# JingyunLiang/HCFlow

Hardware: AMD Instinct MI355X
Metric: HR images/sec (inverse sample) DIV2K x4 160px LR (higher is better)
Workload: dtype f32 via f16x3 split (hi/lo f16 products, f32 accumulate); 1 GPU; SR_DF2K_4X inverse sampling (netG reverse=True), batch 16/GPU, LR 160x160 -> HR 640x640, tau=0.8, eps on device, output all-gather over RCCL for N>1; global_batch=16, lr_size=160, parallelism=dp1, streams_per_gpu=2

## Files before the change

hcflow_amd/csrc/hcf_conv_wino.h:

```cpp
#pragma once
#include <hip/hip_runtime.h>
#include <stdint.h>
#include <string.h>
#include <math.h>
#include <type_traits>
#include <vector>

namespace hcf {
namespace wino {

constexpr int TW = 32, TH = 8, HWP = TW + 2, HHP = TH + 2;
constexpr int A_REAL_PIECES = HHP * HWP * 4;
constexpr int A_BYTES = 22 * 1024;
constexpr int W_BYTES = 16 * 2 * 2 * 32 * 16;
constexpr int STAGE = A_BYTES + W_BYTES;
constexpr int X_BYTES = 10240;
constexpr int S0_OFF = 0, X_OFF = STAGE, S1_OFF = STAGE + X_BYTES, TAB_OFF = S1_OFF + STAGE;
constexpr int LDS_BYTES = TAB_OFF + 512;
constexpr float UNSPLIT = 1.f / 2048.f;

struct Src { const float* p; int cs, c0, n; };
struct Args {
  Src src[3];
  int nsrc;
// ... 48 lines not shown
          memcpy(&pk[o], &p0, 2);
          memcpy(&pk[o + 512], &p1, 2);
        }
    }
  return true;
}

constexpr int W4_BYTES = 65536;
static inline bool pack_weights_wino64(const float* w, int cin, int cout, std::vector<uint16_t>& pk) {
#pragma clang fp contract(off)
  static const double G[4][3] = {{1, 0, 0}, {.5, .5, .5}, {.5, -.5, .5}, {0, 0, 1}};
  if (cout != 64 || (cin & 15)) return false;
  const int nchunk = cin / 16;
  pk.assign(((size_t)nchunk + 1) * (W4_BYTES / 2), 0);
  for (int oc = 0; oc < cout; ++oc)
    for (int ic = 0; ic < cin; ++ic) {
      const float* g = w + ((size_t)oc * cin + ic) * 9;
      double t[4][3], U[4][4];
      for (int i = 0; i < 4; ++i)
        for (int j = 0; j < 3; ++j) t[i][j] = G[i][0] * g[0 * 3 + j] + G[i][1] * g[1 * 3 + j] + G[i][2] * g[2 * 3 + j];
      for (int i = 0; i < 4; ++i)
        for (int j = 0; j < 4; ++j) U[i][j] = t[i][0] * G[j][0] + t[i][1] * G[j][1] + t[i][2] * G[j][2];
      const int nt = oc >> 5, n = oc & 31, c = ic >> 4, h = (ic >> 3) & 1, e = ic & 7;
      for (int xi = 0; xi < 4; ++xi)
        for (int nu = 0; nu < 4; ++nu) {
          const double u = U[xi][nu] * ((xi == 2) ? -1.0 : 1.0) * ((nu == 2) ? -1.0 : 1.0);
          const float x = (float)u;
          if (!(fabsf(x) * 2048.f < 60000.f)) return false;
          const _Float16 hi = (_Float16)x;
          const _Float16 p0 = (_Float16)((float)hi * 2048.f), p1 = (_Float16)((float)((u - (double)(float)hi) * 2048.0));
          const size_t o = (size_t)c * (W4_BYTES / 2) + (size_t)(((xi * 4 + nu) * 2 + nt) * 2) * 512 + (size_t)h * 256 + (size_t)n * 8 + e;
          memcpy(&pk[o], &p0, 2);
          memcpy(&pk[o + 512], &p1, 2);
        }
    }
  return true;
}

constexpr int F1_BYTES = 16384;
static inline bool pack_weights_1x1_frag(const float* w, std::vector<uint16_t>& pk) {
  pk.assign(F1_BYTES / 2, 0);
  for (int mt = 0; mt < 2; ++mt)
    for (int ks = 0; ks < 4; ++ks)
      for (int ln = 0; ln < 64; ++ln)
        for (int e = 0; e < 8; ++e) {
          const int oc = mt * 32 + (ln & 31), ic = 16 * ks + 8 * (ln >> 5) + e;
          const float x = w[oc * 64 + ic];
          if (!(fabsf(x) * 2048.f < 60000.f)) return false;
          const _Float16 hi = (_Float16)x;
          const _Float16 p0 = (_Float16)((float)hi * 2048.f), p1 = (_Float16)((x - (float)hi) * 2048.f);
          const size_t o = ((size_t)((mt * 4 + ks) * 2 + 0) * 64 + ln) * 8 + e;
          memcpy(&pk[o], &p0, 2);
          memcpy(&pk[o + 512], &p1, 2);
        }
  return true;
}

#if defined(__HIPCC__)
typedef float f32x16 __attribute__((ext_vector_type(16)));
typedef float f32x4 __attribute__((ext_vector_type(4)));
typedef _Float16 f16x8 __attribute__((ext_vector_type(8)));
typedef const char __attribute__((address_space(1)))* gcptr;
typedef __attribute__((address_space(3))) void* lptr;

__device__ __forceinline__ int xcd_remap(int orig, int n) {
  const int xcd = orig & 7, q = n >> 3, r = n & 7;
  const int base = (xcd < r) ? xcd * (q + 1) : r * (q + 1) + (xcd - r) * q;
  return base + (orig >> 3);
}
__device__ __forceinline__ gcptr uniform_ptr(const void* p) {
  const uint64_t v = reinterpret_cast<uint64_t>(p);
  const uint32_t lo = __builtin_amdgcn_readfirstlane((uint32_t)v);
  const uint32_t hi = __builtin_amdgcn_readfirstlane((uint32_t)(v >> 32));
  return (gcptr)(((uint64_t)hi << 32) | lo);
}
__device__ __forceinline__ void glds16(gcptr g, char* lds_wave_base) {
  __builtin_amdgcn_global_load_lds((const __attribute__((address_space(1))) void*)g, (lptr)lds_wave_base, 16, 0, 0);
}
__device__ __forceinline__ float act1(float v, float slope, float lo) { return !(v <= 0.f) ? v : slope * fmaxf(v, lo); }
__device__ __forceinline__ int a_off(int px, int part) {
  const int R = px >> 2, sl = (px & 3) * 4 + part;
  return R * 256 + ((sl ^ ((R & 7) << 1)) << 4);
}


namespace v2 {
constexpr int TH2 = 16, HH2 = TH2 + 2;
constexpr int A2_REAL = HH2 * HWP * 4;
constexpr int A2_BYTES = 39 * 1024;
constexpr int STAGE2 = A2_BYTES + W_BYTES;
constexpr int TAB2_OFF = 2 * STAGE2;
constexpr int LDS2_BYTES = TAB2_OFF + 512;
constexpr int FB2_OFF = LDS2_BYTES;
constexpr int LDS2S_BYTES = FB2_OFF + 512 * 16 + 64;
constexpr int ROWB = HWP * 64;
__host__ __device__ constexpr int a2_off(int row, int x, int part) {
  return row * ROWB + (x >> 2) * 256 + (((((x & 3) * 4 + part)) ^ ((x >> 2) & 7)) << 4);
}
}

typedef _Float16 f16x2 __attribute__((ext_vector_type(2)));
typedef uint32_t u32x4 __attribute__((ext_vector_type(4)));
__device__ __forceinline__ void split8(const float (&v)[8], u32x4& h, u32x4& l) {
#pragma unroll
  for (int i = 0; i < 4; ++i) {
    const f16x2 hh = {(_Float16)v[2 * i], (_Float16)v[2 * i + 1]};
    h[i] = __builtin_bit_cast(uint32_t, hh);
    uint32_t lo;
    asm("v_fma_mixlo_f16 %0, %1, -1.0, %2 op_sel_hi:[1,0,0]" : "=v"(lo) : "v"(h[i]), "v"(v[2 * i]));
    asm("v_fma_mixhi_f16 %0, %1, -1.0, %2 op_sel:[1,0,0] op_sel_hi:[1,0,0]" : "+v"(lo) : "v"(h[i]), "v"(v[2 * i + 1]));
    l[i] = lo;
  }
}

__device__ __forceinline__ void split8s(const float (&v)[8], const float s, u32x4& h, u32x4& l) {
#pragma unroll
  for (int i = 0; i < 4; ++i) {
    uint32_t hi, lo;
    asm("v_fma_mixlo_f16 %0, %1, %2, 0 op_sel_hi:[0,0,0]" : "=v"(hi) : "v"(v[2 * i]), "v"(s));
    asm("v_fma_mixhi_f16 %0, %1, %2, 0 op_sel_hi:[0,0,0]" : "+v"(hi) : "v"(v[2 * i + 1]), "v"(s));
    asm("v_fma_mixlo_f16 %0, %1, %2, -%3 op_sel_hi:[0,0,1]" : "=v"(lo) : "v"(v[2 * i]), "v"(s), "v"(hi));
    asm("v_fma_mixhi_f16 %0, %1, %2, -%3 op_sel:[0,0,1] op_sel_hi:[0,0,1]" : "+v"(lo) : "v"(v[2 * i + 1]), "v"(s), "v"(hi));
    h[i] = hi;
    l[i] = lo;
  }
}
__device__ __forceinline__ void input_scales(const float* in_max, float& in_s, float& out_s, int& in_max_bits) {
  in_s = 1.f; out_s = 1.f;
  in_max_bits = __builtin_amdgcn_readfirstlane(__builtin_bit_cast(int, *in_max));
  const float mx = __builtin_bit_cast(float, in_max_bits);
  if (mx > 0.f && mx < 3.0e38f) {
    int ex = 0;
    (void)frexpf(mx, &ex);
    in_s = ldexpf(1.f, 10 - ex);
    out_s = ldexpf(1.f, ex - 10);
  }
  in_s = __builtin_bit_cast(float, __builtin_amdgcn_readfirstlane(__builtin_bit_cast(int, in_s)));
  out_s = __builtin_bit_cast(float, __builtin_amdgcn_readfirstlane(__builtin_bit_cast(int, out_s)));
}

typedef uint32_t u32x2 __attribute__((ext_vector_type(2)));
__device__ __forceinline__ void split4(const f32x4& v, u32x2& h, u32x2& l) {
#pragma unroll
  for (int i = 0; i < 2; ++i) {
    const f16x2 hh = {(_Float16)v[2 * i], (_Float16)v[2 * i + 1]};
    h[i] = __builtin_bit_cast(uint32_t, hh);
    uint32_t lo;
    asm("v_fma_mixlo_f16 %0, %1, -1.0, %2 op_sel_hi:[1,0,0]" : "=v"(lo) : "v"(h[i]), "v"(v[2 * i]));
    asm("v_fma_mixhi_f16 %0, %1, -1.0, %2 op_sel:[1,0,0] op_sel_hi:[1,0,0]" : "+v"(lo) : "v"(h[i]), "v"(v[2 * i + 1]));
    l[i] = lo;
  }
}

template <int RES, bool SC = false>
__global__ __launch_bounds__(512, 1) void conv_wino2_kernel(const Args a, const int nunits) {
  using namespace v2;
  extern __shared__ __attribute__((aligned(16))) char lds[];
  const int tid = threadIdx.x, lane = tid & 63, half = lane >> 5, li = lane & 31;
  const int wave = __builtin_amdgcn_readfirstlane(tid >> 6);
  const int xp = wave & 1, tg = wave >> 1;
  const int H = a.H, W = a.W, ntn = a.ntile_n, nchunk = a.nchunk;
  const int tiles_x = (W + TW - 1) / TW, tiles_y = (H + TH2 - 1) / TH2;

  const bool w7 = (wave == 7);
  const int padpix = a.B * H * W;
  int upix[5];
#pragma unroll
  for (int j = 0; j < 5; ++j) upix[j] = padpix;
  uint32_t partpk = 0;
#pragma unroll
  for (int j = 0; j < 5; ++j) {
    const int pa_ = (8 * j + wave) * 64 + lane, hy_ = (pa_ * 241) >> 15, q_ = pa_ - hy_ * 136, m_ = q_ >> 4;
    partpk |= (uint32_t)(((q_ & 15) ^ (m_ & 7)) & 3) << (4 + 2 * j);
  }
  const int k0 = __builtin_amdgcn_readfirstlane(a.src[0].n >> 4);
  const int k1 = k0 + __builtin_amdgcn_readfirstlane(a.nsrc > 1 ? (a.src[1].n >> 4) : 0);
  const long long npx = (long long)a.B * H * W;
  const __amdgpu_buffer_rsrc_t rs0 = __builtin_amdgcn_make_buffer_rsrc((void*)a.src[0].p, 0, (int)(npx * a.src[0].cs * 4), 0x00020000);
  const __amdgpu_buffer_rsrc_t rs1 = __builtin_amdgcn_make_buffer_rsrc((void*)a.src[a.nsrc > 1 ? 1 : 0].p, 0, (int)(npx * a.src[a.nsrc > 1 ? 1 : 0].cs * 4), 0x00020000);
  const __amdgpu_buffer_rsrc_t rs2 = __builtin_amdgcn_make_buffer_rsrc((void*)a.src[a.nsrc > 2 ? 2 : 0].p, 0, (int)(npx * a.src[a.nsrc > 2 ? 2 : 0].cs * 4), 0x00020000);
  const __amdgpu_buffer_rsrc_t rsw = __builtin_amdgcn_make_buffer_rsrc((void*)a.wpack, 0, (ntn * nchunk + 1) * W_BYTES, 0x00020000);
  const int csb0 = __builtin_amdgcn_readfirstlane(a.src[0].cs) * 4, csb1 = __builtin_amdgcn_readfirstlane(a.src[1].cs) * 4,
            csb2 = __builtin_amdgcn_readfirstlane(a.src[2].cs) * 4;
  const int cb0 = __builtin_amdgcn_readfirstlane(a.src[0].c0) * 4, cb1 = __builtin_amdgcn_readfirstlane(a.src[1].c0) * 4,
            cb2 = __builtin_amdgcn_readfirstlane(a.src[2].c0) * 4;
  const int wvo = lane * 16;

  int ub = 0, uy0 = 0, ux0 = 0, unt = 0, uc = 0;
#define W2_SETUP_UNIT(U)                                                                           \
  {                                                                                                \
    const int v_ = a.rev ? nunits - 1 - xcd_remap((U), nunits) : xcd_remap((U), nunits);           \
    unt = __builtin_amdgcn_readfirstlane(v_ % ntn);                                                \
    const int t_ = v_ / ntn;                                                                       \
    ux0 = __builtin_amdgcn_readfirstlane((t_ % tiles_x) * TW);                                     \
    uy0 = __builtin_amdgcn_readfirstlane(((t_ / tiles_x) % tiles_y) * TH2);                        \
    ub = __builtin_amdgcn_readfirstlane(t_ / (tiles_x * tiles_y));                                 \
    uc = 0;                                                                                        \
    int ln_ = lane;                                                                                \
    asm volatile("" : "+v"(ln_));                                                                  \
    _Pragma("unroll") for (int j = 0; j < 5; ++j) {                                                \
      const int pa_ = (8 * j + wave) * 64 + ln_;            \
      const int hy_ = (pa_ * 241) >> 15;                                \
      const int q_ = pa_ - hy_ * 136, m_ = q_ >> 4;                                                \
      const int hx_ = m_ * 4 + (((q_ & 15) ^ (m_ & 7)) >> 2);                                      \
      const int y = uy0 + hy_ - 1, x = ux0 + hx_ - 1;                                              \
      upix[j] = (hy_ < HH2 && y >= 0 && y < H && x >= 0 && x < W) ? (ub * H + y) * W + x : padpix; \
    }                                                                                              \
  }
#define W2_DMA(RS, VOFF, SOFF, DST) __builtin_amdgcn_raw_ptr_buffer_load_lds((RS), (lptr)(DST), 16, (VOFF), (SOFF), 0, 0)
  int csb_ = 0, so_ = 0, ws_ = 0;
  uint32_t pp_ = partpk;
  __amdgpu_buffer_rsrc_t rsa_ = rs0;
#define W2_CHUNK_SCALARS()                                                                         \
  {                                                                                                \
    const int sidx_ = (uc < k0) ? 0 : (uc < k1) ? 1 : 2;                                           \
    csb_ = sidx_ == 0 ? csb0 : sidx_ == 1 ? csb1 : csb2;                                           \
    rsa_ = sidx_ == 0 ? rs0 : sidx_ == 1 ? rs1 : rs2;                                              \
    so_ = (sidx_ == 0 ? cb0 + uc * 64 : sidx_ == 1 ? cb1 + (uc - k0) * 64 : cb2 + (uc - k1) * 64); \
    ws_ = (unt * nchunk + uc) * W_BYTES;                                                           \
    pp_ = partpk;                                                                                  \
    asm volatile("" : "+v"(pp_));            \
  }
#define W2_A_SLOT(J, DST)                                                                          \
  {                                                                                                \
    const int p16_ = (int)((pp_ >> (2 * (J))) & 0x30u);                                            \
    const int vo_ = (int)__umul24((unsigned)upix[J], (unsigned)csb_) + p16_;                       \
    W2_DMA(rsa_, vo_, so_, DST);                                                                   \
  }
#define W2_ISSUE(J0, J1, STG)                                                                      \
  {                                                                                                \
    char* const sb_ = lds + (STG) * STAGE2 + wave * 1024;                                          \
    _Pragma("unroll") for (int j_ = (J0); j_ < (J1); ++j_) {                                       \
      if (j_ < 4) W2_A_SLOT(j_ < 5 ? j_ : 0, sb_ + j_ * 8192)                                      \
      else if (j_ == 4) { if (!w7) W2_A_SLOT(4, sb_ + 4 * 8192) else W2_DMA(rsw, wvo, ws_, sb_ + 4 * 8192); } \
      else if (j_ < 8) W2_DMA(rsw, wvo, ws_ + (8 * j_ + wave - 39) * 1024, sb_ + j_ * 8192);       \
      else if (!w7) W2_DMA(rsw, wvo, ws_ + (8 * 8 + wave - 39) * 1024, sb_ + 8 * 8192);            \
    }                                                                                              \
  }

  const int trow = li >> 4, tcol = li & 15;
  int poff[4];
#pragma unroll
  for (int j = 0; j < 4; ++j) poff[j] = a2_off(4 * tg + 2 * trow, 2 * tcol + j, 2 * half);
  const int rowP = xp ? ROWB : 0, rowS = xp ? 3 * ROWB : 2 * ROWB;
  const float sg = __builtin_bit_cast(float, __builtin_amdgcn_readfirstlane(__builtin_bit_cast(int, xp ? -1.f : 1.f)));
  const int fw = A2_BYTES + half * 512 + li * 16 + xp * (8 * 4 * 512);

  float in_s = 1.f, out_s = 1.f;
  int in_max_bits = 0;
  if (SC) input_scales(a.in_max, in_s, out_s, in_max_bits);
  constexpr bool FBK = SC && RES == 0;
  const bool fb = FBK && a.fb_y != nullptr;
  if (tid < 64) {
    const float sc_ = (tid < 32 * ntn) ? a.scale[tid] : 1.f, bi_ = (tid < 32 * ntn) ? a.bias[tid] : 0.f;
    reinterpret_cast<float*>(lds + TAB2_OFF)[tid] = bi_ * sc_;
    reinterpret_cast<float*>(lds + TAB2_OFF)[64 + tid] = sc_ * UNSPLIT * out_s;
  }
  if (FBK) {
    if (fb) {
      *reinterpret_cast<f32x4*>(lds + FB2_OFF + tid * 16) = f32x4{0.f, 0.f, 0.f, 0.f};
      if (tid == 0) *reinterpret_cast<int*>(lds + FB2_OFF + 512 * 16) = 0;
    }
  }
  int u = blockIdx.x;
  if (u >= nunits) return;
#if defined(WINO_PROF)
  unsigned long long pw[8] = {0, 0, 0, 0, 0, 0, 0, 0};
  const unsigned long long pw_t0 = __builtin_readcyclecounter();
#endif
  W2_SETUP_UNIT(u)
  W2_CHUNK_SCALARS()
  W2_ISSUE(0, 9, 0)
  ++uc;
  int g = 0;
  const float slope = a.act == 1 ? 0.f : a.act == 2 ? 0.2f : 1.f;

  while (true) {
    f32x16 acc[8];
#pragma unroll
    for (int p = 0; p < 8; ++p)
#pragma unroll
      for (int r = 0; r < 16; ++r) acc[p][r] = 0.f;
    const int eb = ub, ey0 = uy0, ex0 = ux0, ent = unt;
    const int un = u + gridDim.x;

    for (int c = 0; c < nchunk; ++c, ++g) {
      const int stg = g & 1;
#if defined(WINO_PROF)
      const unsigned long long q0 = __builtin_readcyclecounter();
#endif
      asm volatile("s_waitcnt vmcnt(0)" ::: "memory");
#if defined(WINO_PROF)
      const unsigned long long q1 = __builtin_readcyclecounter();
#endif
      __builtin_amdgcn_s_barrier();
#if defined(WINO_PROF)
      const unsigned long long q2 = __builtin_readcyclecounter();
      pw[0] += q1 - q0; pw[1] += q2 - q1;
#endif
      if (c + 1 == nchunk) {
        if (un < nunits) W2_SETUP_UNIT(un)
        else {
          uc = 0; unt = 0;
#pragma unroll
          for (int j = 0; j < 5; ++j) upix[j] = padpix;
        }
      }
      W2_CHUNK_SCALARS()
      const char* const sb = lds + stg * STAGE2;
      const int so = stg ^ 1;
#define W2_LOAD_ROW(D, OFF)                                                                        \
  _Pragma("unroll") for (int j = 0; j < 4; ++j) {                                                  \
    const f32x4 x0_ = *reinterpret_cast<const f32x4*>(sb + poff[j] + (OFF));                       \
    const f32x4 x1_ = *reinterpret_cast<const f32x4*>(sb + (poff[j] ^ 16) + (OFF));                \
    _Pragma("unroll") for (int k = 0; k < 4; ++k) { D[j][k] = x0_[k]; D[j][4 + k] = x1_[k]; }      \
  }
#define W2_V(NU, T, K) (((NU) == 0) ? T[0][K] - T[2][K] : ((NU) == 1) ? T[1][K] + T[2][K] : ((NU) == 2) ? T[1][K] - T[2][K] : T[1][K] - T[3][K])
#define W2_MFMA(P, WW, VX) acc[P] = __builtin_amdgcn_mfma_f32_32x32x16_f16(WW, __builtin_bit_cast(f16x8, VX), acc[P], 0, 0, 0);
#define W2_XI(I, T)                                                                                \
  _Pragma("unroll") for (int nu = 0; nu < 4; ++nu) {                                               \
    float v_[8];                                                                                   \
    _Pragma("unroll") for (int k = 0; k < 8; ++k) v_[k] = W2_V(nu, T, k);                          \
    u32x4 vh_, vl_;                                                                                \
    if (SC) split8s(v_, in_s, vh_, vl_); else split8(v_, vh_, vl_);                                \
    const f16x8 w1_ = *reinterpret_cast<const f16x8*>(sb + fw + (((I) * 4 + nu) * 4) * 512);       \
    const f16x8 w2_ = *reinterpret_cast<const f16x8*>(sb + fw + (((I) * 4 + nu) * 4 + 2) * 512);   \
    W2_MFMA((I) * 4 + nu, w1_, vh_)                                                                \
    W2_MFMA((I) * 4 + nu, w2_, vh_)                                                                \
    W2_MFMA((I) * 4 + nu, w1_, vl_)                                                                \
  }
      float t_[4][8];
      {
        float ra[4][8], rc[4][8];
        W2_LOAD_ROW(ra, rowP)
        W2_LOAD_ROW(rc, 2 * ROWB)
        W2_ISSUE(0, 3, so)
#pragma unroll
        for (int j = 0; j < 4; ++j)
#pragma unroll
          for (int k = 0; k < 8; ++k) t_[j][k] = ra[j][k] - rc[j][k];
      }
      W2_XI(0, t_)
      W2_ISSUE(3, 6, so)
      {
        float ra[4][8], rc[4][8];
        W2_LOAD_ROW(ra, ROWB)
        W2_LOAD_ROW(rc, rowS)
#pragma unroll
        for (int j = 0; j < 4; ++j)
#pragma unroll
          for (int k = 0; k < 8; ++k) t_[j][k] = fmaf(sg, rc[j][k], ra[j][k]);
      }
      W2_ISSUE(6, 9, so)
      ++uc;
      W2_XI(1, t_)
#if defined(WINO_PROF)
      pw[6] += __builtin_readcyclecounter() - q2;
#endif
#undef W2_XI
#undef W2_MFMA
#undef W2_V
#undef W2_LOAD_ROW
    }

#if defined(WINO_PROF)
    const unsigned long long qe0 = __builtin_readcyclecounter();
#endif
    float chk = 0.f;
    f32x4 fbs = {0.f, 0.f, 0.f, 0.f};
    float fbm = 0.f;
    const float fb_neg = a.fb_act == 1 ? 0.f : a.fb_act == 2 ? 0.2f : 1.f;
    {
      char* const xbuf = lds + ((g - 1) & 1) * STAGE2 + tg * 16384;
      const int p8 = lane >> 3, qd = (lane >> 1) & 3, hd = lane & 1;
      const int wpos = (half * 32 + ((li + 4 * half) & 31)) * 16;
      const int wpos1 = (half * 32 + ((li + 4 * half + 8) & 31)) * 16;
      const int cb = ent * 32 + 8 * qd + 4 * hd;
      const f32x4 bs = *reinterpret_cast<const f32x4*>(lds + TAB2_OFF + cb * 4);
      const f32x4 ms = *reinterpret_cast<const f32x4*>(lds + TAB2_OFF + 256 + cb * 4);
      const bool second = (RES == 0) && a.out2 != nullptr && cb >= a.out2_split;
      const float slope_l = second ? (a.act2 == 1 ? 0.f : a.act2 == 2 ? 0.2f : 1.f) : slope;
      __builtin_amdgcn_s_barrier();
#pragma unroll
      for (int oa = 0; oa < 2; ++oa) {
        f32x4 rv1[2][2], rv2[2][2];
        size_t pixs[2][2];
        bool oks[2][2];
        int rpos[2];
#pragma unroll
        for (int sgrp = 0; sgrp < 2; ++sgrp) {
          const int patch = 16 * xp + 8 * sgrp + p8, prow = patch >> 4, pcol = patch & 15;
          rpos[sgrp] = (hd * 32 + ((patch + 4 * hd + 8 * (qd & 1)) & 31)) * 16 + qd * 1024;
#pragma unroll
          for (int ob = 0; ob < 2; ++ob) {
            const int yy = ey0 + 4 * tg + 2 * prow + oa, xx = ex0 + 2 * pcol + ob;
            oks[sgrp][ob] = yy < H && xx < W;
            pixs[sgrp][ob] = (size_t)((size_t)eb * H + (yy < H ? yy : H - 1)) * W + (xx < W ? xx : W - 1);
            if (RES == 1 || RES == 2) rv1[sgrp][ob] = *reinterpret_cast<const f32x4*>(a.res1 + pixs[sgrp][ob] * a.res1_cs + a.res1_c0 + cb);
            if (RES == 2) rv2[sgrp][ob] = *reinterpret_cast<const f32x4*>(a.res2 + pixs[sgrp][ob] * a.res2_cs + a.res2_c0 + cb);
            if (RES == 3) rv1[sgrp][ob] = *reinterpret_cast<const f32x4*>(a.pre + pixs[sgrp][ob] * a.pre_cs + a.pre_c0 + cb);
            if (FBK) { if (fb) rv1[sgrp][ob] = *reinterpret_cast<const f32x4*>(a.fb_y + pixs[sgrp][ob] * a.fb_y_cs + a.fb_y_c0 + cb); }
          }
        }
        if (oa == 1) __builtin_amdgcn_s_barrier();
#pragma unroll
        for (int q = 0; q < 4; ++q) {
          f32x4 P[2];
#pragma unroll
          for (int e = 0; e < 4; ++e) {
            const int r = 4 * q + e;
            float R[2][2];
#pragma unroll
            for (int i = 0; i < 2; ++i) {
              R[i][0] = acc[i * 4 + 0][r] + acc[i * 4 + 1][r] + acc[i * 4 + 2][r];
              R[i][1] = acc[i * 4 + 1][r] - acc[i * 4 + 2][r] - acc[i * 4 + 3][r];
            }
#pragma unroll
            for (int bb = 0; bb < 2; ++bb)
              P[bb][e] = (oa == 0) ? (xp ? R[0][bb] : R[0][bb] + R[1][bb]) : (xp ? -R[0][bb] - R[1][bb] : R[1][bb]);
          }
          char* const wbq = xbuf + ((xp * 2) * 4 + q) * 1024 + ((q & 1) ? wpos1 : wpos);
          *reinterpret_cast<f32x4*>(wbq) = P[0];
          *reinterpret_cast<f32x4*>(wbq + 4096) = P[1];
        }
        __builtin_amdgcn_s_barrier();
#pragma unroll
        for (int sgrp = 0; sgrp < 2; ++sgrp)
#pragma unroll
          for (int ob = 0; ob < 2; ++ob) {
            const f32x4 y0 = *reinterpret_cast<const f32x4*>(xbuf + ((0 * 2 + ob) * 4) * 1024 + rpos[sgrp]);
            const f32x4 y1 = *reinterpret_cast<const f32x4*>(xbuf + ((1 * 2 + ob) * 4) * 1024 + rpos[sgrp]);
            f32x4 v;
#pragma unroll
            for (int e = 0; e < 4; ++e) {
              const float yv = y0[e] + y1[e];
              chk = fmaf(yv, 0.f, chk);
              float z = fmaf(yv, ms[e], bs[e]);
              if (RES == 3) z = fmaf(rv1[sgrp][ob][e], ms[e] * 2048.f, z);
              v[e] = fmaxf(z, slope_l * z);
              if (RES == 1 || RES == 2) v[e] = fmaf(v[e], a.rs1, rv1[sgrp][ob][e]);
              if (RES == 2) v[e] = fmaf(v[e], a.rs2, rv2[sgrp][ob][e]);
            }
            if (FBK) {
              if (fb && oks[sgrp][ob] && cb < a.cout) {
#pragma unroll
                for (int e = 0; e < 4; ++e) {
                  const float yv = rv1[sgrp][ob][e];
                  const bool pos = a.fb_act == 1 ? (yv > 0.f) : (yv >= 0.f);
                  const float dz = (a.fb_act == 0 || pos) ? v[e] : v[e] * fb_neg;
                  v[e] = dz;
                  fbs[e] += dz;
                  fbm = fmaxf(fbm, fabsf(dz));
                }
              }
            }
            if (oks[sgrp][ob] && cb < a.cout) {
              if (second) *reinterpret_cast<f32x4*>(a.out2 + pixs[sgrp][ob] * a.out2_cs + a.out2_c0 + (cb - a.out2_split)) = v;
              else *reinterpret_cast<f32x4*>(a.out + pixs[sgrp][ob] * a.out_cs + a.out_c0 + cb) = v;
            }
          }
      }
    }
    if (__any(chk != chk)) {
      if (lane == 0) atomicOr(a.ovf, 1 | (2 << (eb % 30)));
    }
    if (FBK) {
      if (fb) {
        f32x4* const slot = reinterpret_cast<f32x4*>(lds + FB2_OFF + tid * 16);
        *slot = *slot + fbs;
        if (fbm > 0.f) atomicMax(reinterpret_cast<int*>(lds + FB2_OFF + 512 * 16), __builtin_bit_cast(int, fbm));
      }
    }
#if defined(WINO_PROF)
    pw[3] += __builtin_readcyclecounter() - qe0;
#endif
    u = un;
    if (u >= nunits) break;
  }
  if (FBK) {
    if (fb) {
      asm volatile("s_waitcnt lgkmcnt(0)\n\ts_barrier" ::: "memory");
      if (tid < 32) {
        const int q4 = tid >> 2, e = tid & 3;
        float t0 = 0.f;
        for (int j = 0; j < 64; ++j) t0 += reinterpret_cast<const float*>(lds + FB2_OFF)[(j * 8 + q4) * 4 + e];
        if (tid < a.cout) {
          a.fb_part[((size_t)blockIdx.x * 2 + 0) * a.cout + tid] = t0;
          a.fb_part[((size_t)blockIdx.x * 2 + 1) * a.cout + tid] = 0.f;
        }
      }
      if (tid == 0) {
        const int m = *reinterpret_cast<const int*>(lds + FB2_OFF + 512 * 16), m2 = max(m, in_max_bits);
        if (a.fb_max && m) atomicMax(reinterpret_cast<int*>(a.fb_max), m);
        if (a.fb_max2 && m2) atomicMax(reinterpret_cast<int*>(a.fb_max2), m2);
      }
    }
  }
#if defined(WINO_PROF)
  if (a.dbg && lane == 0 && (blockIdx.x & 31) == 17) {
    atomicAdd(a.dbg + 0, pw[0]); atomicAdd(a.dbg + 1, pw[1]); atomicAdd(a.dbg + 2, __builtin_readcyclecounter() - pw_t0);
    atomicAdd(a.dbg + 3, pw[3]); atomicAdd(a.dbg + 4, 1ull); atomicAdd(a.dbg + 5, pw[5]); atomicAdd(a.dbg + 6, pw[6]);
  }
#endif
#undef W2_SETUP_UNIT
#undef W2_DMA
#undef W2_A_SLOT
#undef W2_ISSUE
#undef W2_CHUNK_SCALARS
}

namespace v4 {
constexpr int TH4 = 8, HH4 = TH4 + 2;
constexpr int A4_BYTES = 22 * 1024;
constexpr int W4L_BYTES = 48 * 1024;
constexpr int W4_OFF0 = 2 * A4_BYTES;
constexpr int X4_SPARE = 19 * 1024;
constexpr int W4_OFF1 = W4_OFF0 + W4L_BYTES + X4_SPARE;
constexpr int TAB4_OFF = W4_OFF1 + W4L_BYTES;
constexpr int LDS4_BYTES = TAB4_OFF + 1024;
constexpr int NPIECE4 = 22 + 48;
}

template <int RES>
__device__ __forceinline__ void wino64_epilogue(const Args& a, char* const lds, const int tab_off, char* const xbase, f32x16 (&acc)[4][2],
                                                const int eb, const int ey0, const int ex0, const int H, const int W, const float slope,
                                                const float slope2, const float slope_f, const int wave, const int lane
#if defined(WINO_PROF)
                                                , unsigned long long* const pw
#endif
                                                ) {
  constexpr bool F1 = (RES == 3);
#if defined(WINO_PROF)
  unsigned long long tl_ = __builtin_readcyclecounter();
#define W64_STAMP(I) { asm volatile("" ::: "memory"); const unsigned long long t_ = __builtin_readcyclecounter(); pw[I] += t_ - tl_; tl_ = t_; asm volatile("" ::: "memory"); }
#else
#define W64_STAMP(I)
#endif
  const int half = lane >> 5, li = lane & 31, xi = wave & 3, tg = wave >> 2;
  (void)li;
  float chk = 0.f;
  char* const xbuf = xbase + tg * 32768;
  const int p8 = lane >> 3, qd = (lane >> 1) & 3, hd = lane & 1;
  const int patch = 8 * xi + p8, prow = patch >> 4, pcol = patch & 15;
  const int wpos = (half * 32 + ((li + 4 * half) & 31)) * 16;
  const int wpos1 = (half * 32 + ((li + 4 * half + 8) & 31)) * 16;
  const int rpos = (hd * 32 + ((patch + 4 * hd + 8 * (qd & 1)) & 31)) * 16 + qd * 1024;
  f32x4 hv[2][2][2];
  const int yy0 = ey0 + 4 * tg + 2 * prow, xx0 = ex0 + 2 * pcol;
  const bool okx1 = xx0 + 1 < W, oky1 = yy0 + 1 < H;
  const bool oks[2][2] = {{yy0 < H && xx0 < W, yy0 < H && okx1}, {oky1 && xx0 < W, oky1 && okx1}};
  const int pix00 = (eb * H + (yy0 < H ? yy0 : H - 1)) * W + (xx0 < W ? xx0 : W - 1);
  const int cb0 = 8 * qd + 4 * hd;
#define W64_PTR(T, BASE, CS, C0, OA, OB) \
  ((T)((BASE) + (ptrdiff_t)pix00 * (CS) + (C0) + cb0) + (((OA) && oky1) ? W * (CS) : 0) + (((OB) && okx1) ? (CS) : 0))
  f32x4 rv1[2][2][2], rv2[2][2][2];
  if (RES == 1 || RES == 2) {
#pragma unroll
    for (int nt = 0; nt < 2; ++nt)
#pragma unroll
      for (int oa = 0; oa < 2; ++oa)
#pragma unroll
        for (int ob = 0; ob < 2; ++ob) {
          rv1[nt][oa][ob] = *reinterpret_cast<const f32x4*>(W64_PTR(const float*, a.res1, a.res1_cs, a.res1_c0, oa, ob) + 32 * nt);
          if (RES == 2) rv2[nt][oa][ob] = *reinterpret_cast<const f32x4*>(W64_PTR(const float*, a.res2, a.res2_cs, a.res2_c0, oa, ob) + 32 * nt);
        }
  }
  __builtin_amdgcn_s_barrier();
  W64_STAMP(8)
#define W64_WRITE(NT, Q)                                                                           \
  {                                                                                                \
    f32x4 Rq[2];                                                                                   \
    _Pragma("unroll") for (int e = 0; e < 4; ++e) {                                                \
      const int r = 4 * (Q) + e;                                                                   \
      Rq[0][e] = acc[0][NT][r] + acc[1][NT][r] + acc[2][NT][r];                                    \
      Rq[1][e] = acc[1][NT][r] - acc[2][NT][r] - acc[3][NT][r];                                    \
    }                                                                                              \
    char* const wbq = xbuf + ((xi * 2) * 4 + (Q)) * 1024 + (((Q) & 1) ? wpos1 : wpos);             \
    *reinterpret_cast<f32x4*>(wbq) = Rq[0];                                                        \
    *reinterpret_cast<f32x4*>(wbq + 4096) = Rq[1];                                                 \
  }
#define W64_READ()                                                                                 \
  _Pragma("unroll") for (int x = 0; x < 4; ++x)                                                    \
    _Pragma("unroll") for (int bb = 0; bb < 2; ++bb) R[x][bb] = *reinterpret_cast<const f32x4*>(xbuf + ((x * 2 + bb) * 4) * 1024 + rpos);
#define W64_MATH(NT, V)                                                                            \
  _Pragma("unroll") for (int oa = 0; oa < 2; ++oa)                                                 \
    _Pragma("unroll") for (int ob = 0; ob < 2; ++ob)                                               \
      _Pragma("unroll") for (int e = 0; e < 4; ++e) {                                              \
        const float yv = oa ? (R[1][ob][e] - R[2][ob][e]) - R[3][ob][e] : (R[0][ob][e] + R[1][ob][e]) + R[2][ob][e]; \
        chk = fmaf(yv, 0.f, chk);                                                                  \
        const float z = fmaf(yv, ms[e], bs[e]);                                                    \
        float v_ = fmaxf(z, slope_t * z);                                                          \
        if (RES == 1 || RES == 2) v_ = fmaf(v_, a.rs1, rv1[NT][oa][ob][e]);                        \
        if (RES == 2) v_ = fmaf(v_, a.rs2, rv2[NT][oa][ob][e]);                                    \
        V[oa][ob][e] = v_;                                                                         \
      }
#define W64_STORE(NT, OA, OB, V) \
  if (oks[OA][OB] && (NT) * 32 + cb0 < a.cout) *reinterpret_cast<f32x4*>(W64_PTR(float*, o_base, o_cs, o_c0, OA, OB)) = V[OA][OB];
  f32x4 R[4][2];
  {
#pragma unroll
    for (int q = 0; q < 4; ++q) W64_WRITE(0, q)
    W64_STAMP(9)
    __builtin_amdgcn_s_barrier();
    W64_STAMP(10)
    W64_READ()
    const f32x4 bs = *reinterpret_cast<const f32x4*>(lds + tab_off + cb0 * 4);
    const f32x4 ms = *reinterpret_cast<const f32x4*>(lds + tab_off + 256 + cb0 * 4);
    const float slope_t = slope;
    float* const o_base = a.out;
    const int o_cs = a.out_cs, o_c0 = a.out_c0;
    (void)o_base; (void)o_cs; (void)o_c0;
    if (!F1) {
      asm volatile("s_waitcnt lgkmcnt(0)" ::: "memory");
      W64_STAMP(11)
      __builtin_amdgcn_s_barrier();
      W64_STAMP(14)
    }
    W64_MATH(0, hv[0])
    if (F1) {
      W64_STAMP(11)
      __builtin_amdgcn_s_barrier();
      W64_STAMP(14)
#pragma unroll
      for (int q = 0; q < 4; ++q) W64_WRITE(1, q)
    } else {
      W64_STAMP(13)
      asm volatile("s_waitcnt vmcnt(0)" ::: "memory");
      if (RES == 1 || RES == 2) {
#pragma unroll
        for (int i = 0; i < 8; ++i) {
          asm volatile("" : "+v"(rv1[i >> 2][(i >> 1) & 1][i & 1]));
          if (RES == 2) asm volatile("" : "+v"(rv2[i >> 2][(i >> 1) & 1][i & 1]));
        }
      }
      W64_STAMP(12)
#pragma unroll
      for (int q = 0; q < 4; ++q) {
        W64_STORE(0, q >> 1, q & 1, hv[0])
        asm volatile("" ::: "memory");
        W64_WRITE(1, q)
        asm volatile("" ::: "memory");
      }
    }
    W64_STAMP(15)
  }
  {
    __builtin_amdgcn_s_barrier();
    W64_STAMP(16)
    W64_READ()
    const f32x4 bs = *reinterpret_cast<const f32x4*>(lds + tab_off + (32 + cb0) * 4);
    const f32x4 ms = *reinterpret_cast<const f32x4*>(lds + tab_off + 256 + (32 + cb0) * 4);
    const bool split_t = a.out2 != nullptr;
    const float slope_t = split_t ? slope2 : slope;
    float* const o_base = split_t ? a.out2 : a.out;
// ... 222 lines not shown
  for (int nu = 0; nu < 4; ++nu) W4_LOAD_W11(nu)
  ++uc;
  int g = 0;
  const float slope = a.act == 1 ? 0.f : a.act == 2 ? 0.2f : 1.f;
  const float slope2 = a.act2 == 1 ? 0.f : a.act2 == 2 ? 0.2f : 1.f;
  const float slope_f = a.f_act == 1 ? 0.f : a.f_act == 2 ? 0.2f : 1.f;

  while (true) {
    f32x16 acc[4][2];
#pragma unroll
    for (int p = 0; p < 4; ++p)
#pragma unroll
      for (int n = 0; n < 2; ++n)
#pragma unroll
        for (int r = 0; r < 16; ++r) acc[p][n][r] = 0.f;
    const int eb = ub, ey0 = uy0, ex0 = ux0;
    const int un = u + gridDim.x;

    for (int c = 0; c < nchunk; ++c, ++g) {
      const int stg = g & 1;
#if defined(WINO_PROF)
      const unsigned long long q0 = __builtin_readcyclecounter();
#endif
      if (c > 0 || g == 0 || a.top_wait) asm volatile("s_waitcnt vmcnt(0)" ::: "memory");
#if defined(WINO_PROF)
      const unsigned long long q1 = __builtin_readcyclecounter();
#endif
      __builtin_amdgcn_s_barrier();
#if defined(WINO_PROF)
      const unsigned long long q2 = __builtin_readcyclecounter();
      pw[0] += q1 - q0; pw[1] += q2 - q1;
      if (c == 0 && g > 0) { pw[21] += q1 - q0; pw[22] += q2 - q1; pw[23] += 1; }
#endif
#pragma unroll
      for (int nu = 0; nu < 4; ++nu) asm volatile("" : "+v"(w11[nu]));
      if (c + 1 == nchunk) {
        if (un < nunits) W4_SETUP_UNIT(un)
        else {
          uc = 0;
#pragma unroll
          for (int j = 0; j < 3; ++j) upix[j] = padpix;
        }
      }
      W4_CHUNK_SCALARS()
      W4_ISSUE_A((g + 1) & 1)
      float t_[4][8];
      {
        const char* const ib = lds + (g & 1) * A4_BYTES;
        float ra[4][8], rb[4][8];
#pragma unroll
        for (int j = 0; j < 4; ++j) {
          const f32x4 x0_ = *reinterpret_cast<const f32x4*>(ib + poff[j] + offA);
          const f32x4 x1_ = *reinterpret_cast<const f32x4*>(ib + (poff[j] ^ 16) + offA);
          const f32x4 y0_ = *reinterpret_cast<const f32x4*>(ib + poff[j] + offB);
          const f32x4 y1_ = *reinterpret_cast<const f32x4*>(ib + (poff[j] ^ 16) + offB);
#pragma unroll
          for (int k = 0; k < 4; ++k) { ra[j][k] = x0_[k]; ra[j][4 + k] = x1_[k]; rb[j][k] = y0_[k]; rb[j][4 + k] = y1_[k]; }
        }
#pragma unroll
        for (int j = 0; j < 4; ++j)
#pragma unroll
          for (int k = 0; k < 8; ++k) t_[j][k] = fmaf(sg, rb[j][k], ra[j][k]);
      }
#if defined(WINO_PROF)
      const unsigned long long q3 = __builtin_readcyclecounter();
      pw[5] += q3 - q2;
#endif
      const char* const wb = lds + (stg ? W4_OFF1 : W4_OFF0) + fw;
#define W4_V(NU, K) (((NU) == 0) ? t_[0][K] - t_[2][K] : ((NU) == 1) ? t_[1][K] + t_[2][K] : ((NU) == 2) ? t_[1][K] - t_[2][K] : t_[1][K] - t_[3][K])
#define W4_MFMA(P, N, WW, VX) acc[P][N] = __builtin_amdgcn_mfma_f32_32x32x16_f16(WW, __builtin_bit_cast(f16x8, VX), acc[P][N], 0, 0, 0);
#pragma unroll
      for (int nu = 0; nu < 4; ++nu) {
        float v_[8];
#pragma unroll
        for (int k = 0; k < 8; ++k) v_[k] = W4_V(nu, k);
        u32x4 vh_, vl_;
        if (SC) split8s(v_, in_s, vh_, vl_); else split8(v_, vh_, vl_);
        const f16x8 w00 = *reinterpret_cast<const f16x8*>(wb + (nu * 3 + 0) * 1024);
        const f16x8 w01 = *reinterpret_cast<const f16x8*>(wb + (nu * 3 + 1) * 1024);
        const f16x8 w10 = *reinterpret_cast<const f16x8*>(wb + (nu * 3 + 2) * 1024);
        W4_MFMA(nu, 0, w00, vh_)
        W4_MFMA(nu, 1, w10, vh_)
        W4_MFMA(nu, 0, w01, vh_)
        W4_MFMA(nu, 1, w11[nu], vh_)
        W4_MFMA(nu, 0, w00, vl_)
        W4_MFMA(nu, 1, w10, vl_)
        if (nu == 0) { W4_ISSUE_W(2, 5, stg ^ 1) }
        else if (nu == 1) { W4_ISSUE_W(5, 7, stg ^ 1) }
        else if (nu == 2) { W4_ISSUE_W(7, 9, stg ^ 1) }
        W4_LOAD_W11(nu)
      }
      ++uc;
#if defined(WINO_PROF)
      pw[6] += __builtin_readcyclecounter() - q3;
#endif
#undef W4_V
#undef W4_MFMA
    }

#if defined(WINO_PROF)
    const unsigned long long qe0 = __builtin_readcyclecounter();
#endif
    int lane_e = lane;
    asm volatile("" : "+v"(lane_e));
    wino64_epilogue<RES>(a, lds, TAB4_OFF, lds + (((g - 1) & 1) ? W4_OFF0 + W4L_BYTES : W4_OFF0), acc, eb, ey0, ex0, H, W, slope, slope2, slope_f, wave, lane_e
#if defined(WINO_PROF)
                         , pw
#endif
                         );
#if defined(WINO_PROF)
    pw[3] += __builtin_readcyclecounter() - qe0;
#endif
    u = un;
    if (u >= nunits) break;
  }
  if (a.clk != nullptr && blockIdx.x == 0 && tid == 0) {
    a.clk[0] += __builtin_readcyclecounter() - a.clk[2];
    a.clk[1] += __builtin_amdgcn_s_memrealtime() - a.clk[3];
  }
#if defined(WINO_PROF)
  if (a.dbg && lane == 0 && (blockIdx.x & 31) == 17) {
    atomicAdd(a.dbg + 0, pw[0]); atomicAdd(a.dbg + 1, pw[1]); atomicAdd(a.dbg + 2, __builtin_readcyclecounter() - pw_t0);
    atomicAdd(a.dbg + 3, pw[3]); atomicAdd(a.dbg + 4, 1ull); atomicAdd(a.dbg + 5, pw[5]); atomicAdd(a.dbg + 6, pw[6]);
    atomicAdd(a.dbg + 7, pw[7]);
    for (int i = 8; i < 24; ++i) atomicAdd(a.dbg + i, pw[i]);
  }
#endif
#undef W4_SETUP_UNIT
#undef W4_DMA
#undef W4_A_SLOT
#undef W4_ISSUE_A
#undef W4_ISSUE_W
#undef W4_LOAD_W11
#undef W4_CHUNK_SCALARS
}


static inline int launch(const Args& a, int ncu, hipStream_t st, int version = 2) {
  if (a.nsrc < 1 || a.nsrc > 3 || !a.wpack || !a.bias || !a.scale || !a.ovf || !a.zeros || !a.out || a.nchunk < 1) return -1;
  if (a.ntile_n < 1 || a.ntile_n > 2 || (a.cout & 3)) return -6;
  int kt = 0;
  for (int i = 0; i < a.nsrc; ++i) {
    if (!a.src[i].p || (a.src[i].n & 15) || (a.src[i].cs & 3) || (a.src[i].c0 & 3) || (reinterpret_cast<uintptr_t>(a.src[i].p) & 15)) return -6;
    if ((long long)a.B * a.H * a.W * a.src[i].cs * 4 >= 0x7fffe000LL) return -6;
    kt += a.src[i].n >> 4;
  }
  if (kt != a.nchunk) return -1;
  if (((a.out_cs | a.out_c0) & 3) || (reinterpret_cast<uintptr_t>(a.out) & 15)) return -6;
  if (a.res1 && (((a.res1_cs | a.res1_c0) & 3) || (reinterpret_cast<uintptr_t>(a.res1) & 15))) return -6;
  if (a.res2 && (((a.res2_cs | a.res2_c0) & 3) || (reinterpret_cast<uintptr_t>(a.res2) & 15))) return -6;
  if (a.res2 && !a.res1) return -1;
  if ((long long)a.B * a.H * a.W >= (1LL << 24)) return -6;
  if (version == 4 && (a.ntile_n != 2 || a.cout > 64)) return -6;
  if (version == 4) {
    const int cs_[4] = {a.out_cs, a.out2 ? a.out2_cs : 0, a.res1 ? a.res1_cs : 0, a.res2 ? a.res2_cs : 0};
    for (int i = 0; i < 4; ++i)
      if (cs_[i] < 0 || (long long)(a.W + 1) * cs_[i] >= 0x7fffffffLL) return -6;
  }
  const int th = (version == 2) ? v2::TH2 : (version == 4) ? v4::TH4 : TH;
  const int tiles_x = (a.W + TW - 1) / TW, tiles_y = (a.H + th - 1) / th;
  const long long nunits = (long long)a.B * tiles_x * tiles_y * (version == 4 ? 1 : a.ntile_n);
  if (nunits < 1 || nunits > 0x7fffffffLL) return -1;
  const unsigned grid = (unsigned)(nunits < ncu ? nunits : ncu);
  static bool attr_dev[64][3][8] = {};
  int dev_ = 0;
  if (hipGetDevice(&dev_) != hipSuccess || dev_ < 0 || dev_ >= 64) return -2;
  bool (&attr)[3][8] = attr_dev[dev_];
  if (a.pre && (version != 2 || a.res1 || a.res2 || ((a.pre_cs | a.pre_c0) & 3) || (reinterpret_cast<uintptr_t>(a.pre) & 15))) return -6;
  if (a.out2 && (a.res1 || a.pre || ((a.out2_cs | a.out2_c0) & 3) || (reinterpret_cast<uintptr_t>(a.out2) & 15))) return -6;
  if (a.out2 && version != 4 && (version != 2 || a.ntile_n != 1 || a.out2_split != 16)) return -6;
  if (a.f_w && (version != 4 || a.res1 || a.res2 || a.out2 || !a.f_bias || !a.f_scale || (reinterpret_cast<uintptr_t>(a.f_w) & 15))) return -6;
  const int res = (a.pre || a.f_w) ? 3 : a.res2 ? 2 : a.res1 ? 1 : 0;
  const bool sc = a.in_max != nullptr;
  if (sc && (res > 1 || a.out2 || (version != 2 && version != 4))) return -6;
  if (a.fb_y && (!sc || version != 2 || res != 0 || a.ntile_n != 1 || !a.fb_part || ((a.fb_y_cs | a.fb_y_c0) & 3) ||
                 (reinterpret_cast<uintptr_t>(a.fb_y) & 15))) return -6;
  const int ldsb = (version == 2) ? (sc ? v2::LDS2S_BYTES : v2::LDS2_BYTES) : (version == 4) ? v4::LDS4_BYTES : LDS_BYTES;
  const int vi = (version == 2) ? 1 : (version == 4) ? 2 : 0;
  const int ai = res + (sc ? 4 : 0);
  auto go = [&](auto fn, int threads) {
    if (!attr[vi][ai]) {
      if (hipFuncSetAttribute(reinterpret_cast<const void*>(fn), hipFuncAttributeMaxDynamicSharedMemorySize, ldsb) != hipSuccess) return -2;
      attr[vi][ai] = true;
    }
    hipLaunchKernelGGL(fn, dim3(grid), dim3(threads), ldsb, st, a, (int)nunits);
    return hipGetLastError() == hipSuccess ? 0 : -2;
  };
  if (sc && version == 4) return res == 0 ? go(conv_wino4_kernel<0, true>, 512) : go(conv_wino4_kernel<1, true>, 512);
  if (sc && version == 2) return res == 0 ? go(conv_wino2_kernel<0, true>, 512) : go(conv_wino2_kernel<1, true>, 512);
  if (version == 4) {
    if (res == 0) return go(conv_wino4_kernel<0>, 512);
    if (res == 1) return go(conv_wino4_kernel<1>, 512);
    if (res == 3) return go(conv_wino4_kernel<3>, 512);
    return go(conv_wino4_kernel<2>, 512);
  }
  if (version == 2) {
    if (res == 0) return go(conv_wino2_kernel<0>, 512);
    if (res == 1) return go(conv_wino2_kernel<1>, 512);
    if (res == 3) return go(conv_wino2_kernel<3>, 512);
    return go(conv_wino2_kernel<2>, 512);
  }
  return -6;
}
#endif

}
}
```

Measured before the change: 136.5 HR images/s.

## Hoist epilogue residual loads before barrier and specialize feedback path at compile time

```diff
diff --git a/hcflow_amd/csrc/hcf_conv_wino.h b/hcflow_amd/csrc/hcf_conv_wino.h
--- a/hcflow_amd/csrc/hcf_conv_wino.h
+++ b/hcflow_amd/csrc/hcf_conv_wino.h
@@ -224,7 +224,7 @@
   }
 }
 
-template <int RES, bool SC = false>
+template <int RES, bool SC = false, bool FB = false>
 __global__ __launch_bounds__(512, 1) void conv_wino2_kernel(const Args a, const int nunits) {
   using namespace v2;
   extern __shared__ __attribute__((aligned(16))) char lds[];
@@ -321,8 +321,8 @@
   float in_s = 1.f, out_s = 1.f;
   int in_max_bits = 0;
   if (SC) input_scales(a.in_max, in_s, out_s, in_max_bits);
-  constexpr bool FBK = SC && RES == 0;
-  const bool fb = FBK && a.fb_y != nullptr;
+  constexpr bool FBK = SC && RES == 0 && FB;
+  constexpr bool fb = FBK;
   if (tid < 64) {
     const float sc_ = (tid < 32 * ntn) ? a.scale[tid] : 1.f, bi_ = (tid < 32 * ntn) ? a.bias[tid] : 0.f;
     reinterpret_cast<float*>(lds + TAB2_OFF)[tid] = bi_ * sc_;
@@ -337,7 +337,9 @@
   int u = blockIdx.x;
   if (u >= nunits) return;
 #if defined(WINO_PROF)
-  unsigned long long pw[8] = {0, 0, 0, 0, 0, 0, 0, 0};
+  unsigned long long pw[48];
+#pragma unroll
+  for (int i = 0; i < 48; ++i) pw[i] = 0;
   const unsigned long long pw_t0 = __builtin_readcyclecounter();
 #endif
   W2_SETUP_UNIT(u)
@@ -361,7 +363,7 @@
 #if defined(WINO_PROF)
       const unsigned long long q0 = __builtin_readcyclecounter();
 #endif
-      asm volatile("s_waitcnt vmcnt(0)" ::: "memory");
+      if (c > 0 || g == 0) asm volatile("s_waitcnt vmcnt(0)" ::: "memory");
 #if defined(WINO_PROF)
       const unsigned long long q1 = __builtin_readcyclecounter();
 #endif
@@ -369,6 +371,7 @@
 #if defined(WINO_PROF)
       const unsigned long long q2 = __builtin_readcyclecounter();
       pw[0] += q1 - q0; pw[1] += q2 - q1;
+      if (c == 0 && g > 0) { pw[44] += q1 - q0; pw[45] += q2 - q1; pw[46] += 1; }
 #endif
       if (c + 1 == nchunk) {
         if (un < nunits) W2_SETUP_UNIT(un)
@@ -437,6 +440,10 @@
 
 #if defined(WINO_PROF)
     const unsigned long long qe0 = __builtin_readcyclecounter();
+    unsigned long long tl_ = qe0;
+#define W2_STAMP(I) { asm volatile("" ::: "memory"); const unsigned long long t_ = __builtin_readcyclecounter(); pw[I] += t_ - tl_; tl_ = t_; asm volatile("" ::: "memory"); }
+#else
+#define W2_STAMP(I)
 #endif
     float chk = 0.f;
     f32x4 fbs = {0.f, 0.f, 0.f, 0.f};
@@ -444,37 +451,52 @@
     const float fb_neg = a.fb_act == 1 ? 0.f : a.fb_act == 2 ? 0.2f : 1.f;
     {
       char* const xbuf = lds + ((g - 1) & 1) * STAGE2 + tg * 16384;
-      const int p8 = lane >> 3, qd = (lane >> 1) & 3, hd = lane & 1;
-      const int wpos = (half * 32 + ((li + 4 * half) & 31)) * 16;
-      const int wpos1 = (half * 32 + ((li + 4 * half + 8) & 31)) * 16;
+      int le = lane;
+      asm volatile("" : "+v"(le));
+      const int p8 = le >> 3, qd = (le >> 1) & 3, hd = le & 1;
+      const int half_e = le >> 5, li_e = le & 31;
+      const int wpos = (half_e * 32 + ((li_e + 4 * half_e) & 31)) * 16;
+      const int wpos1 = (half_e * 32 + ((li_e + 4 * half_e + 8) & 31)) * 16;
       const int cb = ent * 32 + 8 * qd + 4 * hd;
       const f32x4 bs = *reinterpret_cast<const f32x4*>(lds + TAB2_OFF + cb * 4);
       const f32x4 ms = *reinterpret_cast<const f32x4*>(lds + TAB2_OFF + 256 + cb * 4);
-      const bool second = (RES == 0) && a.out2 != nullptr && cb >= a.out2_split;
+      const bool second = (RES == 0) && !SC && a.out2 != nullptr && cb >= a.out2_split;
       const float slope_l = second ? (a.act2 == 1 ? 0.f : a.act2 == 2 ? 0.2f : 1.f) : slope;
+      const int yy0 = ey0 + 4 * tg + 2 * xp, xx0 = ex0 + 2 * p8;
+      const bool oky[2] = {yy0 < H, yy0 + 1 < H};
+      const bool okx[2][2] = {{xx0 < W, xx0 + 1 < W}, {xx0 + 16 < W, xx0 + 17 < W}};
+      int rpos[2];
+#pragma unroll
+      for (int sgrp = 0; sgrp < 2; ++sgrp) rpos[sgrp] = (hd * 32 + ((16 * xp + 8 * sgrp + p8 + 4 * hd + 8 * (qd & 1)) & 31)) * 16 + qd * 1024;
+      const int pix00 = (eb * H + (oky[0] ? yy0 : H - 1)) * W + (okx[0][0] ? xx0 : W - 1);
+#define W2_PTR(T, BASE, CS, C0, OA, SG, OB) \
+  ((T)((BASE) + (ptrdiff_t)pix00 * (CS) + (C0) + cb) + (((OA) && oky[1]) ? W * (CS) : 0) + (okx[SG][OB] ? (16 * (SG) + (OB)) * (CS) : 0))
+      float* const o_base = second ? a.out2 : a.out;
+      const int o_cs = second ? a.out2_cs : a.out_cs, o_c0 = second ? a.out2_c0 - a.out2_split : a.out_c0;
+      f32x4 rv1[2][2][2], rv2[2][2][2];
+#define W2_RES_LOAD(OA)                                                                            \
+  _Pragma("unroll") for (int sgrp = 0; sgrp < 2; ++sgrp)                                           \
+    _Pragma("unroll") for (int ob = 0; ob < 2; ++ob) {                                             \
+      if (RES == 1 || RES == 2) rv1[OA][sgrp][ob] = *reinterpret_cast<const f32x4*>(W2_PTR(const float*, a.res1, a.res1_cs, a.res1_c0, OA, sgrp, ob)); \
+      if (RES == 2) rv2[OA][sgrp][ob] = *reinterpret_cast<const f32x4*>(W2_PTR(const float*, a.res2, a.res2_cs, a.res2_c0, OA, sgrp, ob)); \
+      if (RES == 3) rv1[OA][sgrp][ob] = *reinterpret_cast<const f32x4*>(W2_PTR(const float*, a.pre, a.pre_cs, a.pre_c0, OA, sgrp, ob)); \
+      if (FBK) rv1[OA][sgrp][ob] = *reinterpret_cast<const f32x4*>(W2_PTR(const float*, a.fb_y, a.fb_y_cs, a.fb_y_c0, OA, sgrp, ob)); \
+    }
+#define W2_RES_LANDED(OA)                                                                          \
+  _Pragma("unroll") for (int sgrp = 0; sgrp < 2; ++sgrp)                                           \
+    _Pragma("unroll") for (int ob = 0; ob < 2; ++ob) {                                             \
+      if (RES >= 1 || FBK) asm volatile("" : "+v"(rv1[OA][sgrp][ob]));                             \
+      if (RES == 2) asm volatile("" : "+v"(rv2[OA][sgrp][ob]));                                    \
+    }
+      W2_RES_LOAD(0) W2_RES_LOAD(1)
       __builtin_amdgcn_s_barrier();
+      W2_STAMP(32)
 #pragma unroll
       for (int oa = 0; oa < 2; ++oa) {
-        f32x4 rv1[2][2], rv2[2][2];
-        size_t pixs[2][2];
-        bool oks[2][2];
-        int rpos[2];
-#pragma unroll
-        for (int sgrp = 0; sgrp < 2; ++sgrp) {
-          const int patch = 16 * xp + 8 * sgrp + p8, prow = patch >> 4, pcol = patch & 15;
-          rpos[sgrp] = (hd * 32 + ((patch + 4 * hd + 8 * (qd & 1)) & 31)) * 16 + qd * 1024;
-#pragma unroll
-          for (int ob = 0; ob < 2; ++ob) {
-            const int yy = ey0 + 4 * tg + 2 * prow + oa, xx = ex0 + 2 * pcol + ob;
-            oks[sgrp][ob] = yy < H && xx < W;
-            pixs[sgrp][ob] = (size_t)((size_t)eb * H + (yy < H ? yy : H - 1)) * W + (xx < W ? xx : W - 1);
-            if (RES == 1 || RES == 2) rv1[sgrp][ob] = *reinterpret_cast<const f32x4*>(a.res1 + pixs[sgrp][ob] * a.res1_cs + a.res1_c0 + cb);
-            if (RES == 2) rv2[sgrp][ob] = *reinterpret_cast<const f32x4*>(a.res2 + pixs[sgrp][ob] * a.res2_cs + a.res2_c0 + cb);
-            if (RES == 3) rv1[sgrp][ob] = *reinterpret_cast<const f32x4*>(a.pre + pixs[sgrp][ob] * a.pre_cs + a.pre_c0 + cb);
-            if (FBK) { if (fb) rv1[sgrp][ob] = *reinterpret_cast<const f32x4*>(a.fb_y + pixs[sgrp][ob] * a.fb_y_cs + a.fb_y_c0 + cb); }
-          }
-        }
-        if (oa == 1) __builtin_amdgcn_s_barrier();
+        if (oa == 1) {
+          __builtin_amdgcn_s_barrier();
+          W2_STAMP(38)
+        }
 #pragma unroll
         for (int q = 0; q < 4; ++q) {
           f32x4 P[2];
@@ -495,29 +517,44 @@
           *reinterpret_cast<f32x4*>(wbq) = P[0];
           *reinterpret_cast<f32x4*>(wbq + 4096) = P[1];
         }
+        W2_STAMP(oa ? 39 : 33)
         __builtin_amdgcn_s_barrier();
+        W2_STAMP(oa ? 40 : 34)
+        f32x4 y0[2][2], y1[2][2];
 #pragma unroll
         for (int sgrp = 0; sgrp < 2; ++sgrp)
 #pragma unroll
           for (int ob = 0; ob < 2; ++ob) {
-            const f32x4 y0 = *reinterpret_cast<const f32x4*>(xbuf + ((0 * 2 + ob) * 4) * 1024 + rpos[sgrp]);
-            const f32x4 y1 = *reinterpret_cast<const f32x4*>(xbuf + ((1 * 2 + ob) * 4) * 1024 + rpos[sgrp]);
+            y0[sgrp][ob] = *reinterpret_cast<const f32x4*>(xbuf + ((0 * 2 + ob) * 4) * 1024 + rpos[sgrp]);
+            y1[sgrp][ob] = *reinterpret_cast<const f32x4*>(xbuf + ((1 * 2 + ob) * 4) * 1024 + rpos[sgrp]);
+          }
+        W2_STAMP(oa ? 41 : 35)
+        if (oa == 0) {
+          asm volatile("s_waitcnt vmcnt(0)" ::: "memory");
+          W2_RES_LANDED(0) W2_RES_LANDED(1)
+        }
+        W2_STAMP(oa ? 42 : 36)
+#pragma unroll
+        for (int sgrp = 0; sgrp < 2; ++sgrp)
+#pragma unroll
+          for (int ob = 0; ob < 2; ++ob) {
             f32x4 v;
 #pragma unroll
             for (int e = 0; e < 4; ++e) {
-              const float yv = y0[e] + y1[e];
+              const float yv = y0[sgrp][ob][e] + y1[sgrp][ob][e];
               chk = fmaf(yv, 0.f, chk);
               float z = fmaf(yv, ms[e], bs[e]);
-              if (RES == 3) z = fmaf(rv1[sgrp][ob][e], ms[e] * 2048.f, z);
+              if (RES == 3) z = fmaf(rv1[oa][sgrp][ob][e], ms[e] * 2048.f, z);
               v[e] = fmaxf(z, slope_l * z);
-              if (RES == 1 || RES == 2) v[e] = fmaf(v[e], a.rs1, rv1[sgrp][ob][e]);
-              if (RES == 2) v[e] = fmaf(v[e], a.rs2, rv2[sgrp][ob][e]);
+              if (RES == 1 || RES == 2) v[e] = fmaf(v[e], a.rs1, rv1[oa][sgrp][ob][e]);
+              if (RES == 2) v[e] = fmaf(v[e], a.rs2, rv2[oa][sgrp][ob][e]);
             }
+            const bool ok = oky[oa] && okx[sgrp][ob] && cb < a.cout;
             if (FBK) {
-              if (fb && oks[sgrp][ob] && cb < a.cout) {
+              if (fb && ok) {
 #pragma unroll
                 for (int e = 0; e < 4; ++e) {
-                  const float yv = rv1[sgrp][ob][e];
+                  const float yv = rv1[oa][sgrp][ob][e];
                   const bool pos = a.fb_act == 1 ? (yv > 0.f) : (yv >= 0.f);
                   const float dz = (a.fb_act == 0 || pos) ? v[e] : v[e] * fb_neg;
                   v[e] = dz;
@@ -526,13 +563,15 @@
                 }
               }
             }
-            if (oks[sgrp][ob] && cb < a.cout) {
-              if (second) *reinterpret_cast<f32x4*>(a.out2 + pixs[sgrp][ob] * a.out2_cs + a.out2_c0 + (cb - a.out2_split)) = v;
-              else *reinterpret_cast<f32x4*>(a.out + pixs[sgrp][ob] * a.out_cs + a.out_c0 + cb) = v;
-            }
+            if (ok) *reinterpret_cast<f32x4*>(W2_PTR(float*, o_base, o_cs, o_c0, oa, sgrp, ob)) = v;
           }
-      }
-    }
+        W2_STAMP(oa ? 43 : 37)
+      }
+#undef W2_PTR
+#undef W2_RES_LOAD
+#undef W2_RES_LANDED
+    }
+#undef W2_STAMP
     if (__any(chk != chk)) {
       if (lane == 0) atomicOr(a.ovf, 1 | (2 << (eb % 30)));
     }
@@ -572,6 +611,7 @@
   if (a.dbg && lane == 0 && (blockIdx.x & 31) == 17) {
     atomicAdd(a.dbg + 0, pw[0]); atomicAdd(a.dbg + 1, pw[1]); atomicAdd(a.dbg + 2, __builtin_readcyclecounter() - pw_t0);
     atomicAdd(a.dbg + 3, pw[3]); atomicAdd(a.dbg + 4, 1ull); atomicAdd(a.dbg + 5, pw[5]); atomicAdd(a.dbg + 6, pw[6]);
+    for (int i = 32; i < 47; ++i) atomicAdd(a.dbg + i, pw[i]);
   }
 #endif
 #undef W2_SETUP_UNIT
@@ -1100,10 +1140,11 @@
   if (a.res2 && !a.res1) return -1;
   if ((long long)a.B * a.H * a.W >= (1LL << 24)) return -6;
   if (version == 4 && (a.ntile_n != 2 || a.cout > 64)) return -6;
-  if (version == 4) {
-    const int cs_[4] = {a.out_cs, a.out2 ? a.out2_cs : 0, a.res1 ? a.res1_cs : 0, a.res2 ? a.res2_cs : 0};
-    for (int i = 0; i < 4; ++i)
-      if (cs_[i] < 0 || (long long)(a.W + 1) * cs_[i] >= 0x7fffffffLL) return -6;
+  if (version == 4 || version == 2) {
+    const int span = version == 4 ? a.W + 1 : a.W + 17;
+    const int cs_[6] = {a.out_cs, a.out2 ? a.out2_cs : 0, a.res1 ? a.res1_cs : 0, a.res2 ? a.res2_cs : 0, a.pre ? a.pre_cs : 0, a.fb_y ? a.fb_y_cs : 0};
+    for (int i = 0; i < 6; ++i)
+      if (cs_[i] < 0 || (long long)span * cs_[i] >= 0x7fffffffLL) return -6;
   }
   const int th = (version == 2) ? v2::TH2 : (version == 4) ? v4::TH4 : TH;
   const int tiles_x = (a.W + TW - 1) / TW, tiles_y = (a.H + th - 1) / th;
@@ -1125,8 +1166,8 @@
                  (reinterpret_cast<uintptr_t>(a.fb_y) & 15))) return -6;
   const int ldsb = (version == 2) ? (sc ? v2::LDS2S_BYTES : v2::LDS2_BYTES) : (version == 4) ? v4::LDS4_BYTES : LDS_BYTES;
   const int vi = (version == 2) ? 1 : (version == 4) ? 2 : 0;
-  const int ai = res + (sc ? 4 : 0);
-  auto go = [&](auto fn, int threads) {
+  auto go = [&](auto fn, int threads, int ai_ = -1) {
+    const int ai = ai_ >= 0 ? ai_ : res + (sc ? 4 : 0);
     if (!attr[vi][ai]) {
       if (hipFuncSetAttribute(reinterpret_cast<const void*>(fn), hipFuncAttributeMaxDynamicSharedMemorySize, ldsb) != hipSuccess) return -2;
       attr[vi][ai] = true;
@@ -1135,6 +1176,7 @@
     return hipGetLastError() == hipSuccess ? 0 : -2;
   };
   if (sc && version == 4) return res == 0 ? go(conv_wino4_kernel<0, true>, 512) : go(conv_wino4_kernel<1, true>, 512);
+  if (sc && version == 2 && a.fb_y) return go(conv_wino2_kernel<0, true, true>, 512, 6);
   if (sc && version == 2) return res == 0 ? go(conv_wino2_kernel<0, true>, 512) : go(conv_wino2_kernel<1, true>, 512);
   if (version == 4) {
     if (res == 0) return go(conv_wino4_kernel<0>, 512);
```

Result: no change. 137.0 HR images/s (median of 6 runs) (+0.4%).
